# dpbriggs/Distributed-Sieve-e

Hardware: AMD Instinct MI355X
Metric: sieved integers/sec at N=1e11, 1/2/4/8 MI355X; % of LDS/HBM roofline (higher is better)
Workload: dtype u32; 1 GPU; N=1e+11 odd-only chunked sieve, P=1 spread-work chunks (one per GPU), mask resident in HBM; N=100000000000, P=1, cs=49999999999, mask_bytes_per_gpu=6250000000, parallelism=range-partition x1 (RCCL broadcast + all-reduce)

## Files before the change

distributed-sieve-e_amd/csrc/dse_wheel_geometry.h:

```cpp
#pragma once
#include <hip/hip_runtime.h>
#include <stddef.h>
#include <stdint.h>

#include <algorithm>

#include "dse_internal.h"

namespace dse {
namespace {

constexpr uint32_t KP = 1u << kWheelLogKP;
constexpr uint32_t BLOCKS = KP / 32;
constexpr uint32_t IMG_WORDS = 8 * BLOCKS;
constexpr uint32_t IMG_BYTES = 4 * IMG_WORDS;
static_assert(IMG_BYTES == KP, "a period index is its block's byte address");
#define DSE_IMG_OFF_S "32768"
constexpr uint32_t kImgOff = 32768;
#define DSE_STR2(x) #x
#define DSE_STR(x) DSE_STR2(x)
constexpr uint32_t NT = 1024;
constexpr uint32_t NW = NT / 64;
static_assert(BLOCKS % (64 * NW) == 0, "expansion blocks");
#ifndef DSE_TA
#define DSE_TA 96
#endif
constexpr uint32_t TA = DSE_TA;
#ifndef DSE_TB1
#define DSE_TB1 640
#endif
constexpr uint32_t TB1 = DSE_TB1;
#ifndef DSE_TB
#define DSE_TB 1536
#endif
constexpr uint32_t TB = DSE_TB;
static_assert(TA <= 256 && TA < TB1 && TB1 <= TB && TB <= KP / 8, "unit thresholds");
static_assert(KP / (128 * (TA + 1)) <= 10 && KP / (32 * (TB1 + 1)) <= 10, "class_marks_k covers K <= 10");
constexpr uint32_t kMidCap = TB >= 16384 ? 1920 : TB >= 8192 ? 1040 : TB >= 4096 ? 580 : 320;
constexpr uint32_t kOutWordsPerSeg = (uint32_t)(kWheelOutBits / 32);

constexpr uint32_t kQMax = 79;

constexpr uint32_t inv30_const(uint32_t q) {
  for (uint32_t x = 1; x < q; ++x)
    if ((30 * x) % q == 1) return x;
  return 0;
}
constexpr int kNG = 9;
constexpr uint32_t kGQ[kNG][3] = {{7, 11, 13}, {17, 19, 1}, {23, 29, 1}, {31, 37, 1}, {41, 43, 1},
                                  {47, 53, 1}, {59, 61, 1}, {67, 71, 1}, {73, 79, 1}};
constexpr uint32_t gmod(int g) { return kGQ[g][0] * kGQ[g][1] * kGQ[g][2]; }
constexpr uint32_t kInitWords = IMG_WORDS / NT;
constexpr uint32_t kInitRun = 32 * kInitWords;
constexpr uint32_t kExpandBlocks = BLOCKS / NW;
constexpr uint32_t kInitBlocks = kInitRun / 128 + 2;
constexpr uint32_t gdw(int g) { return ((gmod(g) + 32 * (4 * kInitBlocks + 1) + 127) / 128) * 4; }
constexpr uint32_t gbase(int g) { return g == 0 ? 0u : gbase(g - 1) + gdw(g - 1); }
constexpr uint32_t kGDW = gbase(kNG);
constexpr uint32_t kGInv30[kNG] = {inv30_const(gmod(0)), inv30_const(gmod(1)), inv30_const(gmod(2)),
                                   inv30_const(gmod(3)), inv30_const(gmod(4)), inv30_const(gmod(5)),
                                   inv30_const(gmod(6)), inv30_const(gmod(7)), inv30_const(gmod(8))};

struct InitTables {
  uint32_t w[4 * kGDW];
};
constexpr InitTables make_init_tables() {
  InitTables t{};
  for (int g = 0; g < kNG; ++g) {
    for (uint32_t j = 0; j < gdw(g) + 3; ++j) {
      uint32_t v = 0;
      for (uint32_t b = 0; b < 32; ++b) {
        const uint32_t y = 32 * j + b;
        const bool hit = y % kGQ[g][0] == 0 || y % kGQ[g][1] == 0 || (kGQ[g][2] > 1 && y % kGQ[g][2] == 0);
        v |= (uint32_t)hit << b;
      }
      for (uint32_t k = 0; k < 4; ++k)
        if (j >= k && j - k < gdw(g)) t.w[k * kGDW + gbase(g) + (j - k)] = v;
    }
  }
  return t;
}
__device__ const InitTables g_init_tables = make_init_tables();

constexpr uint32_t kLPieces = 16;
constexpr uint32_t kMaxRanges = 9;

}


struct WheelRange {
  uint64_t V0;
  uint64_t nbits;
  uint64_t KB0;
  uint64_t rho_pack;
  uint32_t* out;
  unsigned long long* count;
  uint32_t pl_pack;
  uint32_t e_iota;
  uint64_t fix;
  uint32_t seg0;
  uint16_t v0g[kNG];
  uint32_t lsh;
  uint32_t lcap[kLPieces];
  uint32_t variant;
};

struct WheelArgs {
  WheelRange r[kMaxRanges];
  uint32_t nranges;
  uint32_t nseg;
  uint32_t nthr[5];
  const uint32_t* bk_entries;
  const uint32_t* bk_start;
  const uint32_t* bk_reg0;
  const uint32_t* bk_n0;
  const unsigned long long* bk_spill;
  const uint32_t* bk_nspill;
  uint64_t bk_spill_cap;
  uint32_t bk_k0;
};
static_assert(sizeof(WheelArgs) <= 4096, "kernel arguments");
static_assert(alignof(WheelArgs) <= 8, "kernel argument layout");

namespace {

constexpr uint32_t kWaOffset = 8;

#ifndef DSE_BK_GRID
#define DSE_BK_GRID 1024
#endif
#ifndef DSE_BK_UNIT_BATCHES
#define DSE_BK_UNIT_BATCHES 4
#endif
constexpr uint32_t kBkBatchU = 16;
constexpr uint32_t kBkUnit = 64 * kBkBatchU * DSE_BK_UNIT_BATCHES;
constexpr uint32_t kBkGrid0 = DSE_BK_GRID;
#ifndef DSE_BK0_LISTS
#define DSE_BK0_LISTS 16
#endif
constexpr uint32_t kBk0Lists = DSE_BK0_LISTS;
static_assert(kBkGrid0 % kBk0Lists == 0 && 64 % kBk0Lists == 0, "band-0 bucket units");
constexpr uint32_t kKeyShift = 20;
static_assert(IMG_WORDS * 32 <= (1u << kKeyShift), "bucket entry layout");

}
}
```

distributed-sieve-e_amd/csrc/dse_wheel_kernel.h:

```cpp
#pragma once
#include <type_traits>

#include "dse_expand_bits.h"
#include "dse_wheel_geometry.h"

namespace dse {
namespace {

__device__ __forceinline__ uint32_t lds_addr(const uint32_t* p) {
  return (uint32_t)(uintptr_t)(const __attribute__((address_space(3))) uint32_t*)p;
}

__device__ __forceinline__ void lds_drain() { asm volatile("s_waitcnt lgkmcnt(0)" ::: "memory"); }

__device__ __forceinline__ uint32_t opaque(uint32_t x) {
  asm volatile("" : "+v"(x));
  return x;
}

constexpr uint32_t kBlockMask = ~31u;
#ifndef DSE_FAKE_CF_L
#define DSE_FAKE_CF_L 0
#endif
constexpr uint32_t kBlockMaskL = DSE_FAKE_CF_L ? ~127u : kBlockMask;
#ifndef DSE_FAKE_CF_INIT
#define DSE_FAKE_CF_INIT 0
#endif
#ifndef DSE_SHORT_TAIL
#define DSE_SHORT_TAIL 16
#endif
constexpr uint32_t kShortTail = DSE_SHORT_TAIL;
constexpr uint32_t odd_primes_upto(uint32_t x) {
  uint32_t c = 0;
  for (uint32_t v = 3; v <= x; v += 2) {
    bool pr = true;
    for (uint32_t d = 3; d * d <= v; d += 2)
      if (v % d == 0) { pr = false; break; }
    c += pr;
  }
  return c;
}
constexpr uint32_t kL0 = odd_primes_upto(TB);
constexpr uint32_t kLPrimeMask = 0x800FFFFFu;
static_assert(kWheelMaxPrime <= (1u << 20), "pl[] words: the L primes (odd, <= kWheelMaxPrime) are below 2^20");
__host__ __device__ constexpr uint32_t l_plan(uint32_t pmin, uint32_t pmax, uint32_t kp) {
  if (pmin > kp) return 2;
  if (pmin > kp / 2) return 1;
  const uint32_t n_min = pmax >= kp ? 0u : kp / pmax;
  const uint32_t n_all = (kp + pmin - 1) / pmin;
  return n_all - n_min <= kShortTail ? n_all << 3 : 4u | n_min << 3;
}
static_assert(l_plan(TB + 2, TB + 2, 1u << 17) < (1u << 11) && l_plan(TB + 2, TB + 2, 1u << 16) < (1u << 11),
              "the plan fits bits 20..30 of a pl[] word (bit 31: kLPrimeMask's dead-lane flag)");
static_assert(odd_primes_upto(kQMax) + kMidCap >= kL0, "the L list starts at kL0 whenever it exists");

__device__ __forceinline__ void mark_k(uint32_t pb4, uint32_t k, uint32_t one) {
  uint32_t a, b;
  asm volatile(
      "v_and_or_b32 %0, %2, %3, %4\n\t"
      "v_lshlrev_b32 %1, %2, %5\n\t"
      "ds_or_b32 %0, %1 offset:" DSE_IMG_OFF_S
      : "=&v"(a), "=&v"(b)
      : "v"(k), "s"(kBlockMask), "v"(pb4), "v"(one)
      : "memory");
}

__device__ __forceinline__ void mark_k_step(uint32_t pb4, uint32_t& k, uint32_t p, uint32_t one) {
  uint32_t a, b;
  asm volatile(
      "v_and_or_b32 %0, %2, %3, %4\n\t"
      "v_lshlrev_b32 %1, %2, %6\n\t"
      "ds_or_b32 %0, %1 offset:" DSE_IMG_OFF_S "\n\t"
      "v_add_u32 %2, %2, %5"
      : "=&v"(a), "=&v"(b), "+v"(k)
      : "s"(kBlockMask), "v"(pb4), "v"(p), "v"(one)
      : "memory");
}

__device__ __forceinline__ void mark_k_step4(uint32_t pb4, uint32_t& k, uint32_t p, uint32_t one) {
  uint32_t a0, b0, a1, b1;
  asm volatile(
      "v_and_or_b32 %0, %4, %5, %6\n\t"
      "v_lshlrev_b32 %1, %4, %8\n\t"
      "v_add_u32 %4, %4, %7\n\t"
      "ds_or_b32 %0, %1 offset:" DSE_IMG_OFF_S "\n\t"
      "v_and_or_b32 %2, %4, %5, %6\n\t"
      "v_lshlrev_b32 %3, %4, %8\n\t"
      "v_add_u32 %4, %4, %7\n\t"
      "ds_or_b32 %2, %3 offset:" DSE_IMG_OFF_S "\n\t"
      "v_and_or_b32 %0, %4, %5, %6\n\t"
      "v_lshlrev_b32 %1, %4, %8\n\t"
      "v_add_u32 %4, %4, %7\n\t"
      "ds_or_b32 %0, %1 offset:" DSE_IMG_OFF_S "\n\t"
      "v_and_or_b32 %2, %4, %5, %6\n\t"
      "v_lshlrev_b32 %3, %4, %8\n\t"
      "v_add_u32 %4, %4, %7\n\t"
      "ds_or_b32 %2, %3 offset:" DSE_IMG_OFF_S
      : "=&v"(a0), "=&v"(b0), "=&v"(a1), "=&v"(b1), "+v"(k)
      : "s"(kBlockMask), "v"(pb4), "v"(p), "v"(one)
      : "memory");
}


__device__ __forceinline__ uint32_t mark_run(uint32_t pb4, uint32_t k, uint32_t p, uint32_t n, uint32_t one) {
  uint32_t h = 0;
  for (; h + 4 <= n; h += 4) mark_k_step4(pb4, k, p, one);
  for (; h < n; ++h) mark_k_step(pb4, k, p, one);
  return k;
}

__device__ __forceinline__ void mark_tail(uint32_t pb4, uint32_t k, uint32_t p, uint32_t one) {
  uint64_t sv;
  uint32_t a, b;
  asm volatile(
      "s_mov_b64 %3, exec\n\t"
      "v_cmpx_gt_u32_e32 vcc, %5, %2\n\t"
      "s_cbranch_execz 2f\n"
      "1:\n\t"
      "v_and_or_b32 %0, %2, %6, %7\n\t"
      "v_lshlrev_b32 %1, %2, %8\n\t"
      "v_add_u32 %2, %2, %4\n\t"
      "ds_or_b32 %0, %1 offset:" DSE_IMG_OFF_S "\n\t"
      "v_cmpx_gt_u32_e32 vcc, %5, %2\n\t"
      "s_cbranch_execnz 1b\n"
      "2:\n\t"
      "s_mov_b64 exec, %3"
      : "=&v"(a), "=&v"(b), "+v"(k), "=&s"(sv)
      : "v"(p), "s"(KP), "s"(kBlockMask), "v"(pb4), "v"(one)
      : "memory", "vcc");
}

__device__ __forceinline__ void mark_at(uint32_t a, uint32_t bit) {
  asm volatile("ds_or_b32 %0, %1 offset:" DSE_IMG_OFF_S : : "v"(a), "v"(bit) : "memory");
}

template <int K>
__device__ __forceinline__ void class_marks(uint32_t pb4, uint32_t k, uint32_t p, uint32_t D, uint32_t one) {
#pragma unroll 1
  for (uint32_t r = 0; r < 32; ++r) {
    uint32_t a, b;
    asm volatile(
        "v_and_or_b32 %0, %2, %3, %4\n\t"
        "v_lshlrev_b32 %1, %2, %5\n\t"
        "ds_or_b32 %0, %1 offset:" DSE_IMG_OFF_S
        : "=&v"(a), "=&v"(b)
        : "v"(k), "s"(kBlockMask), "v"(pb4), "v"(one)
        : "memory");
#pragma unroll
    for (int t = 1; t < K; ++t) {
      a += D;
      mark_at(a, b);
    }
    k = opaque(k + p);
  }
}
__device__ __forceinline__ void class_marks_k(uint32_t K, uint32_t pb4, uint32_t k, uint32_t p, uint32_t D,
                                              uint32_t one) {
  switch (K) {
    case 0: return;
    case 1: class_marks<1>(pb4, k, p, D, one); return;
    case 2: class_marks<2>(pb4, k, p, D, one); return;
    case 3: class_marks<3>(pb4, k, p, D, one); return;
    case 4: class_marks<4>(pb4, k, p, D, one); return;
    case 5: class_marks<5>(pb4, k, p, D, one); return;
    case 6: class_marks<6>(pb4, k, p, D, one); return;
    case 7: class_marks<7>(pb4, k, p, D, one); return;
    case 8: class_marks<8>(pb4, k, p, D, one); return;
    case 9: class_marks<9>(pb4, k, p, D, one); return;
    case 10: class_marks<10>(pb4, k, p, D, one); return;
    default: __builtin_unreachable();
  }
}

__host__ __device__ __forceinline__ uint32_t mod_barrett(uint64_t x, uint32_t p, uint64_t m) {
#if defined(__HIP_DEVICE_COMPILE__)
  uint64_t q = __umul64hi(x, m);
#else
  uint64_t q = (uint64_t)(((unsigned __int128)x * m) >> 64);
#endif
  uint64_t r = x - q * p;
  if (r >= p) r -= p;
  if (r >= p) r -= p;
  return (uint32_t)r;
}

__device__ __forceinline__ uint64_t barrett_factor(uint32_t p) {
  const double dp = (double)p;
  uint64_t m = (uint64_t)(18446744073709551615.0 / dp);
  if (m > ~0ull / 2) m = ~0ull / 2;
  int64_t r = (int64_t)(~0ull - m * (uint64_t)p);
  m += (int64_t)__builtin_floor((double)r / dp);
  r = (int64_t)(~0ull - m * (uint64_t)p);
  while (r < 0) { --m; r += p; }
  while (r >= (int64_t)p) { ++m; r -= p; }
  return m;
}

__device__ __forceinline__ float fast_rcp(float x) { return __builtin_amdgcn_rcpf(x); }

__device__ __forceinline__ uint32_t div_ceil_small(uint32_t t, uint32_t p, float invp) {
  uint32_t q = (uint32_t)((float)t * invp);
  q = q * p > t ? q - 1 : q;
  q = (q + 1) * p <= t ? q + 1 : q;
  return q + (q * p != t ? 1u : 0u);
}

__device__ __forceinline__ uint32_t div_small(uint32_t t, uint32_t p, float invp) {
  uint32_t q = (uint32_t)((float)t * invp);
  q = q * p > t ? q - 1 : q;
  q = (q + 1) * p <= t ? q + 1 : q;
  return q;
}

__device__ __forceinline__ uint32_t mulmod_small(uint32_t x, uint32_t y, uint32_t p, float invp) {
  const uint32_t xy = x * y;
  uint32_t q = (uint32_t)((float)xy * invp);
  int32_t r = (int32_t)(xy - q * p);
  r = r < 0 ? r + (int32_t)p : r;
  r = r < 0 ? r + (int32_t)p : r;
  r = r >= (int32_t)p ? r - (int32_t)p : r;
  r = r >= (int32_t)p ? r - (int32_t)p : r;
  return (uint32_t)r;
}

__host__ __device__ __forceinline__ uint64_t inv30_of(uint64_t p) {
  constexpr uint64_t T = (14ull << 0) | (8ull << 12) | (9ull << 20) | (11ull << 24) | (3ull << 32) | (5ull << 36) |
                         (6ull << 44) | (0ull << 56);
  const uint32_t r = (uint32_t)(p % 30u);
  const uint64_t a = 2 * ((T >> (4 * (r >> 1))) & 15) + 1;
  return (p * a + 1) / 30;
}

__device__ __forceinline__ uint32_t plane_first(uint32_t Xs, uint32_t rho, uint32_t p, uint32_t inv30,
                                                float invp) {
  uint32_t t = Xs + rho;
  t = t >= p ? t - p : t;
  const uint32_t u = t ? p - t : 0u;
  return mulmod_small(u, inv30, p, invp);
}

__device__ __forceinline__ uint32_t first_at_or_after(uint32_t kp, uint32_t start, uint32_t p, float invp) {
  if (start <= kp) return kp;
  return kp + p * div_ceil_small(start - kp, p, invp);
}

__device__ __forceinline__ uint32_t kmin_for(uint32_t D, uint32_t rho) {
  return D > rho ? (D - rho + 29u) / 30u : 0u;
}


template <int K>
__device__ __forceinline__ void a_classes(uint32_t pb4, uint32_t k, uint32_t p, uint32_t one) {
  const uint32_t D = p << 8;
#pragma unroll 1
  for (uint32_t r = 0; r < 32; ++r) {
    uint32_t a, bit;
    asm volatile(
        "v_and_or_b32 %0, %2, %3, %4\n\t"
        "v_lshlrev_b32 %1, %2, %5"
        : "=&v"(a), "=&v"(bit)
        : "v"(k), "s"(kBlockMask), "v"(pb4), "v"(one));
#pragma unroll
    for (int t = 0; t < K; ++t) {
      mark_at(a, bit);
      a += D;
    }
    mark_at(a, bit);
    k = opaque(k + p);
  }
}

struct MidRes {
  uint32_t* x;
  const uint32_t* inc;
  bool have;
};
__device__ __forceinline__ uint32_t mid_residue(const MidRes& mr, uint32_t i, uint32_t p, uint64_t m, uint64_t Vs,
                                                bool writer) {
  const uint32_t xs = mr.have ? mr.x[i] : mod_barrett(Vs, p, m);
  if (writer) {
    const uint32_t t = xs + mr.inc[i];
    mr.x[i] = min(t, t - p);
  }
  return xs;
}

__device__ __forceinline__ void unit_A(uint32_t img0, uint32_t pi, uint64_t m, const MidRes& mr, uint32_t idx,
                                       uint64_t Vs, uint64_t rho_pack, uint32_t lane, uint32_t one) {
  const uint32_t p = pi & 0xFFFFu, inv30 = pi >> 16;
  const uint64_t p2 = (uint64_t)p * p;
  const uint32_t Xs = __builtin_amdgcn_readfirstlane(mid_residue(mr, idx, p, m, Vs, lane == 0));
  const float invp = fast_rcp((float)p);
  const uint32_t pl = lane & 7, c = lane >> 3;
  const uint32_t rho = (uint32_t)(rho_pack >> (5 * pl)) & 31u;
  const uint32_t kp = plane_first(Xs, rho, p, inv30, invp);
  const uint32_t pb4 = img0 + 4 * pl;
  const uint32_t k = kp + 32 * c * p;
  if (p2 <= Vs) {
    switch (KP / (256 * p)) {
      case 1: a_classes<1>(pb4, k, p, one); return;
      case 2: a_classes<2>(pb4, k, p, one); return;
      case 3: a_classes<3>(pb4, k, p, one); return;
      case 4: a_classes<4>(pb4, k, p, one); return;
      case 5: a_classes<5>(pb4, k, p, one); return;
      case 6: a_classes<6>(pb4, k, p, one); return;
      case 7: a_classes<7>(pb4, k, p, one); return;
      default: __builtin_unreachable();
    }
  }
  const uint32_t kmin = kmin_for((uint32_t)(p2 - Vs), rho);
  for (uint32_t r = 0; r < 32; ++r)
    for (uint32_t kk = k + r * p; kk < KP; kk += 256 * p)
      if (kk >= kmin) mark_k(pb4, kk, one);
}

__device__ __forceinline__ void unit_B1(uint32_t img0, const uint32_t* __restrict__ s_mid_p,
                                        const uint64_t* __restrict__ s_mid_m, const MidRes& mr, uint32_t j0,
                                        uint32_t nj, uint64_t Vs, uint64_t rho_pack, uint32_t lane, uint32_t one) {
  const uint32_t h = lane >> 5, pl = lane & 7, j = (lane >> 3) & 3;
  if (h >= nj) return;
  const uint32_t pi = s_mid_p[j0 + h];
  const uint32_t p = pi & 0xFFFFu, inv30 = pi >> 16;
  const uint64_t m = s_mid_m[j0 + h];
  const float invp = fast_rcp((float)p);
  const uint32_t rho = (uint32_t)(rho_pack >> (5 * pl)) & 31u;
  const uint32_t kp = plane_first(mid_residue(mr, j0 + h, p, m, Vs, (lane & 31) == 0), rho, p, inv30, invp);
  const uint32_t pb4 = img0 + 4 * pl;
  uint32_t k = kp + 32 * j * p;
  const uint64_t p2 = (uint64_t)p * p;
  if (p2 > Vs) {
    const uint32_t kmin = kmin_for((uint32_t)min(p2 - Vs, (uint64_t)0xFFFFFFFFu), rho);
    for (; k < KP; k += 96 * p)
      for (uint32_t r = 0; r < 32 && k < KP; ++r, k += p)
        if (k >= kmin) mark_k(pb4, k, one);
    return;
  }
  const uint32_t pmax = __builtin_amdgcn_readlane(p, nj == 2 ? 32 : 0);
  const uint32_t tf = (KP / pmax) / 128;
  class_marks_k(tf, pb4, k, p, 128 * p, one);
  k += tf * (128 * p);
  const uint32_t pmin = __builtin_amdgcn_readfirstlane(p);
  const uint32_t n_all = __builtin_amdgcn_readfirstlane(div_ceil_small(KP, pmin, fast_rcp((float)pmin)));
  for (uint32_t base = 128 * tf; base < n_all; base += 128) {
    mark_run(pb4, k, p, min(32u, n_all - base), one);
    k += 128 * p;
  }
}

__device__ __forceinline__ void unit_B2(uint32_t img0, const uint32_t* __restrict__ s_mid_p,
                                        const uint64_t* __restrict__ s_mid_m, const MidRes& mr, uint32_t j0,
                                        uint32_t nj, uint64_t Vs, uint64_t Vend, uint64_t rho_pack, uint32_t lane,
                                        uint32_t one) {
  const uint32_t pl = lane & 7, jp = lane >> 3;
  const bool valid = jp < nj;
  const uint32_t pi = s_mid_p[valid ? j0 + jp : j0];
  const uint32_t p = pi & 0xFFFFu, inv30 = pi >> 16;
  const uint64_t m = s_mid_m[valid ? j0 + jp : j0];
  const float invp = fast_rcp((float)p);
  const uint32_t rho = (uint32_t)(rho_pack >> (5 * pl)) & 31u;
  uint32_t k = plane_first(mid_residue(mr, valid ? j0 + jp : j0, p, m, Vs, valid && pl == 0), rho, p, inv30, invp);
  const uint64_t p2 = (uint64_t)p * p;
  const bool slow = p2 > Vs;
  if (slow) k = p2 >= Vend ? KP : first_at_or_after(k, kmin_for((uint32_t)(p2 - Vs), rho), p, invp);
  const uint32_t pmax = __builtin_amdgcn_readfirstlane(s_mid_p[j0 + nj - 1]) & 0xFFFFu;
  const bool any_slow = __builtin_amdgcn_ballot_w64(slow) != 0;
  const uint32_t n_u = any_slow ? 0u : KP / pmax;
  const uint32_t pb4 = img0 + 4 * pl;
  if (!valid) return;
  const uint32_t K = n_u / 32;
  class_marks_k(K, pb4, k, p, 32 * p, one);
  k += K * (32 * p);
  if (any_slow) {
    mark_tail(pb4, mark_run(pb4, k, p, n_u - 32 * K, one), p, one);
    return;
  }
  const uint32_t pmin = __builtin_amdgcn_readfirstlane(s_mid_p[j0]) & 0xFFFFu;
  const uint32_t n_all = __builtin_amdgcn_readfirstlane(div_ceil_small(KP, pmin, fast_rcp((float)pmin)));
  mark_run(pb4, k, p, n_all - 32 * K, one);
}

struct LargeOps {
  uint32_t p;
  uint64_t m;
  uint32_t a[8];
};

__device__ __forceinline__ void load_L(LargeOps& o, const uint32_t* __restrict__ P, const uint64_t* __restrict__ M,
                                       const uint32_t* __restrict__ A, uint32_t il, uint32_t np, bool need_m) {
  const uint32_t ic = min(il, np - 1);
  o.p = il < np ? *reinterpret_cast<const uint32_t*>(reinterpret_cast<const char*>(P) + (ic << 2)) : 0xFFFFFFFFu;
  o.m = need_m ? M[ic] : 0ull;
  const uint4* row = reinterpret_cast<const uint4*>(reinterpret_cast<const char*>(A) + (ic << 5));
  const uint4 lo = row[0], hi = row[1];
  o.a[0] = lo.x; o.a[1] = lo.y; o.a[2] = lo.z; o.a[3] = lo.w;
  o.a[4] = hi.x; o.a[5] = hi.y; o.a[6] = hi.z; o.a[7] = hi.w;
}

__device__ __forceinline__ void undef_ops(LargeOps& o) {
  asm volatile("" : "=v"(o.p), "=v"(o.m), "=v"(o.a[0]), "=v"(o.a[1]), "=v"(o.a[2]), "=v"(o.a[3]), "=v"(o.a[4]),
               "=v"(o.a[5]), "=v"(o.a[6]), "=v"(o.a[7]));
}

__device__ __forceinline__ void mark_entry(uint32_t img0, uint32_t e, uint32_t one) {
  uint32_t a, b;
  asm volatile(
      "v_lshrrev_b32 %0, 3, %2\n\t"
      "v_and_or_b32 %0, %0, -4, %4\n\t"
      "v_lshlrev_b32 %1, %2, %3\n\t"
      "ds_or_b32 %0, %1 offset:" DSE_IMG_OFF_S
      : "=&v"(a), "=&v"(b)
      : "v"(e), "v"(one), "v"(img0)
      : "memory");
}

constexpr uint64_t kQuotBits = 22;
constexpr uint64_t kQuotErr38 = (1ull << (38 - 22)) / (TB + 1) + 1;
static_assert((1ull << 32) / (TB + 1) < (1ull << kQuotBits), "Kb < 2^32: float quotient within 1 (and < 2^24 for __umul24)");
static_assert((kQuotErr38 + 2) * kWheelMaxPrime < (1ull << 31), "Kb < 2^38: the rest Kb - q p must be exact in int32");
static_assert(kWheelMaxPrime < (1ull << 23), "__mul24 / __umul24 operands and float-exact p");
static_assert((uint64_t)(kWheelMaxPrime + 1) * (kWheelMaxPrime + 1) / 30 < (1ull << 38),
              "ranges without bucketed primes never need the Barrett path (unit_L<false>)");

__device__ __forceinline__ uint32_t kb_mod_p_f32(uint32_t kb, uint32_t p, float invp) {
  const uint32_t q = (uint32_t)((float)kb * invp);
  uint32_t qp;
  asm("v_mul_u32_u24 %0, %1, %2" : "=v"(qp) : "v"(q), "v"(p));
  uint32_t x = kb - qp;
  x = min(x, x + p);
  return min(x, x - p);
}

__device__ __forceinline__ uint32_t kb_mod_p_f38(uint64_t Kb, uint32_t p, float invp) {
  const uint32_t q = (uint32_t)((float)Kb * invp);
  const int32_t r = (int32_t)((uint32_t)Kb - q * p);
  const int32_t q2 = (int32_t)((float)r * invp);
  uint32_t x = (uint32_t)(r - __mul24(q2, (int32_t)p));
  x = min(x, x + p);
  return min(x, x - p);
}

template <bool BARRETT>
__device__ __forceinline__ uint32_t kb_mod_p(uint64_t Kb, uint32_t p, float invp, uint64_t m) {
  if (Kb < (1ull << 32)) return kb_mod_p_f32((uint32_t)Kb, p, invp);
  if (!BARRETT || Kb < (1ull << 38)) return kb_mod_p_f38(Kb, p, invp);
  return mod_barrett(Kb, p, m);
}

struct PlaneSteps {
  uint32_t pb[8];
  uint32_t ne[8];
  uint32_t one;
};

__device__ __forceinline__ uint32_t plane_start(uint32_t a, uint32_t nKbm, uint32_t ne, uint32_t p) {
  uint32_t t, u;
  asm("v_add3_u32 %0, %2, %3, %4\n\t"
      "v_add_u32 %1, %0, %5\n\t"
      "v_min_u32 %0, %0, %1"
      : "=&v"(t), "=&v"(u)
      : "v"(a), "v"(nKbm), "v"(ne), "v"(p));
  return t;
}

#define DSE_PLANE_START(A, NE)                                       \
  "v_add3_u32 %0, " A ", %15, " NE "\n\t"  \
  "v_add_u32 %1, %0, %16\n\t"                                        \
  "v_min_u32 %0, %0, %1\n\t"
#define DSE_PLANE_MARK(PB)               \
  "v_and_or_b32 %1, %0, %17, " PB "\n\t" \
  "v_lshlrev_b32 %2, %0, %18\n\t"        \
  "ds_or_b32 %1, %2 offset:" DSE_IMG_OFF_S "\n\t"
#define DSE_PLANE_NEXT "v_add_u32 %0, %0, %16\n\t"
template <int NM>
__device__ __forceinline__ void start_marks4(const uint32_t* a, const uint32_t* ne, const uint32_t* pb, uint32_t nKbm,
                                             uint32_t p, uint32_t one) {
  uint32_t t, u, b;
  if (NM == 1)
    asm volatile(
        DSE_PLANE_START("%3", "%7") DSE_PLANE_MARK("%11")
        DSE_PLANE_START("%4", "%8") DSE_PLANE_MARK("%12")
        DSE_PLANE_START("%5", "%9") DSE_PLANE_MARK("%13")
        DSE_PLANE_START("%6", "%10") DSE_PLANE_MARK("%14")
        : "=&v"(t), "=&v"(u), "=&v"(b)
        : "v"(a[0]), "v"(a[1]), "v"(a[2]), "v"(a[3]), "v"(ne[0]), "v"(ne[1]), "v"(ne[2]), "v"(ne[3]), "v"(pb[0]),
          "v"(pb[1]), "v"(pb[2]), "v"(pb[3]), "v"(nKbm), "v"(p), "s"(kBlockMaskL), "v"(one)
        : "memory");
  else
    asm volatile(
        DSE_PLANE_START("%3", "%7") DSE_PLANE_MARK("%11") DSE_PLANE_NEXT DSE_PLANE_MARK("%11")
        DSE_PLANE_START("%4", "%8") DSE_PLANE_MARK("%12") DSE_PLANE_NEXT DSE_PLANE_MARK("%12")
        DSE_PLANE_START("%5", "%9") DSE_PLANE_MARK("%13") DSE_PLANE_NEXT DSE_PLANE_MARK("%13")
        DSE_PLANE_START("%6", "%10") DSE_PLANE_MARK("%14") DSE_PLANE_NEXT DSE_PLANE_MARK("%14")
        : "=&v"(t), "=&v"(u), "=&v"(b)
        : "v"(a[0]), "v"(a[1]), "v"(a[2]), "v"(a[3]), "v"(ne[0]), "v"(ne[1]), "v"(ne[2]), "v"(ne[3]), "v"(pb[0]),
          "v"(pb[1]), "v"(pb[2]), "v"(pb[3]), "v"(nKbm), "v"(p), "s"(kBlockMaskL), "v"(one)
        : "memory");
}

#ifndef DSE_LOCKSTEP
#define DSE_LOCKSTEP 1
#endif
#define DSE_MARK8_ONE(A, B, K, PB)                   \
  "v_and_or_b32 " A ", " K ", %21, " PB "\n\t"     \
  "v_lshlrev_b32 " B ", " K ", %22\n\t"             \
  "v_add_u32 " K ", " K ", %20\n\t"                 \
  "ds_or_b32 " A ", " B " offset:" DSE_IMG_OFF_S "\n\t"
__device__ __forceinline__ void mark8(uint32_t (&k)[8], const uint32_t* pb, uint32_t p, uint32_t one) {
  uint32_t a0, b0, a1, b1;
  asm volatile(DSE_MARK8_ONE("%0", "%1", "%4", "%12") DSE_MARK8_ONE("%2", "%3", "%5", "%13")
                   DSE_MARK8_ONE("%0", "%1", "%6", "%14") DSE_MARK8_ONE("%2", "%3", "%7", "%15")
                       DSE_MARK8_ONE("%0", "%1", "%8", "%16") DSE_MARK8_ONE("%2", "%3", "%9", "%17")
                           DSE_MARK8_ONE("%0", "%1", "%10", "%18") DSE_MARK8_ONE("%2", "%3", "%11", "%19")
               : "=&v"(a0), "=&v"(b0), "=&v"(a1), "=&v"(b1), "+v"(k[0]), "+v"(k[1]), "+v"(k[2]), "+v"(k[3]),
                 "+v"(k[4]), "+v"(k[5]), "+v"(k[6]), "+v"(k[7])
               : "v"(pb[0]), "v"(pb[1]), "v"(pb[2]), "v"(pb[3]), "v"(pb[4]), "v"(pb[5]), "v"(pb[6]), "v"(pb[7]),
                 "v"(p), "s"(kBlockMaskL), "v"(one)
               : "memory");
}

template <int MODE, bool TAIL = false>
__device__ __forceinline__ void unit_L_fast(const LargeOps& o, uint32_t p, uint32_t nKbm, const PlaneSteps& ps,
                                            uint32_t n_run) {
  if (MODE != 0) {
    constexpr int NM = MODE == 2 ? 1 : 2;
    start_marks4<NM>(o.a, ps.ne, ps.pb, nKbm, p, ps.one);
    start_marks4<NM>(o.a + 4, ps.ne + 4, ps.pb + 4, nKbm, p, ps.one);
    return;
  }
#if DSE_LOCKSTEP
  if (!TAIL) {
    uint32_t kk[8];
#pragma unroll
    for (uint32_t q = 0; q < 8; ++q) kk[q] = plane_start(o.a[q], nKbm, ps.ne[q], p);
#pragma unroll 1
    for (uint32_t h = 0; h < n_run; ++h) mark8(kk, ps.pb, p, ps.one);
    return;
  }
#endif
#pragma unroll
  for (uint32_t q = 0; q < 8; ++q) {
    const uint32_t kk = plane_start(o.a[q], nKbm, ps.ne[q], p);
    const uint32_t pb4 = ps.pb[q];
    const uint32_t k = mark_run(pb4, kk, p, n_run, ps.one);
    if (TAIL) mark_tail(pb4, k, p, ps.one);
  }
}

template <bool BARRETT>
__device__ __forceinline__ void unit_L(const LargeOps& o, uint64_t Vs, uint64_t Vend, uint64_t Kb,
                                       const PlaneSteps& ps, uint32_t pl_rot, const uint64_t* rho_pack_p,
                                       uint32_t sqrt_vs) {
  const uint32_t p = o.p & kLPrimeMask;
  const float invp = fast_rcp((float)p);
  const uint32_t kbm = kb_mod_p<BARRETT>(Kb, p, invp, o.m);
  const uint32_t nKbm = 0u - kbm;
  const uint32_t pmax = __builtin_amdgcn_readlane(p, 63);
  const bool none = pmax > sqrt_vs;
  if (!none) {
    const uint32_t plan = (uint32_t)__builtin_amdgcn_readfirstlane(o.p) >> 20;
    const uint32_t n_run = plan >> 3;
    if ((plan & 3) == 2) unit_L_fast<2>(o, p, nKbm, ps, 0);
    else if ((plan & 3) == 1) unit_L_fast<1>(o, p, nKbm, ps, 0);
    else if (!(plan & 4)) unit_L_fast<0>(o, p, nKbm, ps, n_run);
    else unit_L_fast<0, true>(o, p, nKbm, ps, n_run);
    return;
  }
  const uint32_t pmin = __builtin_amdgcn_readfirstlane(p);
  const uint64_t p2 = (uint64_t)p * p;
  const bool live = p2 < Vend;
  const bool slow = p2 > Vs;
  const uint32_t D = slow && live ? (uint32_t)(p2 - Vs) : 0u;
  if (!live) return;
  const uint64_t rho_pack = *(volatile const uint64_t*)rho_pack_p;
#pragma unroll
  for (uint32_t q = 0; q < 8; ++q) {
    uint32_t kk = plane_start(o.a[q], nKbm, ps.ne[q], p);
    if (slow) {
      const uint32_t pl = (pl_rot >> (3 * q)) & 7u;
      const uint32_t rho = (uint32_t)(rho_pack >> (5 * pl)) & 31u;
      const uint32_t kmin = kmin_for(D, rho);
      if (kmin > kk) {
        const uint32_t d = kmin - kk;
        uint32_t qd = (uint32_t)((float)d * invp);
        while (qd * p < d) ++qd;
        while (qd > 0 && (qd - 1) * p >= d) --qd;
        kk += qd * p;
      }
    }
    const uint32_t pb4 = ps.pb[q];
    if (pmin > KP / 2) {
      mark_k(pb4, kk, ps.one);
      mark_k(pb4, kk + p, ps.one);
    } else {
      for (; kk < KP; kk += p) mark_k(pb4, kk, ps.one);
    }
  }
}

struct WheelLdsLow {
  uint64_t mid_m[kMidCap];
  uint32_t mid_p[kMidCap];
  uint32_t mid_x[kMidCap];
  uint32_t mid_inc[kMidCap];
  uint32_t x_seg;
  uint4 itab[kGDW];
  uint32_t thr[5];
  uint32_t ctr;
  unsigned long long rcnt[kMaxRanges];
};
static_assert(sizeof(WheelLdsLow) <= kImgOff, "LDS below the image");
struct WheelLds : WheelLdsLow {
  uint8_t pad[kImgOff - sizeof(WheelLdsLow)];
  uint32_t img[IMG_WORDS];
};
static_assert(sizeof(WheelLds) == kImgOff + IMG_BYTES, "the image ends the allocation");

template <bool BK>
__global__ __launch_bounds__(NT) void wheel_segments_kernel(const void* __restrict__ table, WheelArgs wa) {
  __shared__ WheelLds lds;
  uint64_t* const s_mid_m = lds.mid_m;
  uint32_t* const s_mid_p = lds.mid_p;
  uint32_t* const s_thr = lds.thr;

  const TableHeader* th = reinterpret_cast<const TableHeader*>(table);
  const uint32_t np = th->count;
  const uint32_t* __restrict__ P = reinterpret_cast<const uint32_t*>(reinterpret_cast<const char*>(table) + 16);
  const uint64_t* __restrict__ M =
      reinterpret_cast<const uint64_t*>(reinterpret_cast<const char*>(table) + table_m_offset(th->cap));
  const uint32_t* __restrict__ A =
      reinterpret_cast<const uint32_t*>(reinterpret_cast<const char*>(table) + table_a_offset(th->cap));
  const uint32_t* __restrict__ PL = reinterpret_cast<const uint32_t*>(reinterpret_cast<const char*>(table) +
                                                                    table_l_offset(th->cap)) +
                                    (kWheelLogKP == 17 ? 0u : th->cap);

#if defined(DSE_PAD_NOPS) && DSE_PAD_NOPS > 0
  asm volatile(".rept " DSE_STR(DSE_PAD_NOPS) "\n\ts_nop 0\n\t.endr");
#endif
  const uint32_t tid = threadIdx.x, lane_id = tid & 63, wave = tid >> 6;

  if (tid == 0) {
    s_thr[0] = min(wa.nthr[0], np);
    s_thr[1] = min(wa.nthr[1], np);
    s_thr[2] = min(wa.nthr[2], np);
    s_thr[3] = min(min(wa.nthr[3], np), s_thr[0] + kMidCap);
    s_thr[2] = min(s_thr[2], s_thr[3]);
    s_thr[4] = max(s_thr[3], min(wa.nthr[4], np));
    lds.ctr = 0;
    lds.x_seg = ~0u;
  }
  if (tid < kMaxRanges) lds.rcnt[tid] = 0;
  for (uint32_t idx = tid; idx < 4 * kGDW; idx += NT) reinterpret_cast<uint32_t*>(lds.itab)[idx] = g_init_tables.w[idx];
  __syncthreads();
  const uint32_t i_mid0 = s_thr[0], i_midB = s_thr[1], i_midB2 = s_thr[2], i_mid1 = s_thr[3];
  for (uint32_t i = tid; i < i_mid1 - i_mid0; i += NT) {
    const uint32_t q = P[i_mid0 + i];
    s_mid_p[i] = q | ((uint32_t)inv30_of(q) << 16);
    s_mid_m[i] = M[i_mid0 + i];
    lds.mid_inc[i] = (uint32_t)(((uint64_t)gridDim.x * kWheelSpan) % q);
  }
  const uint32_t nA = i_midB - i_mid0;
  const uint32_t n_mid = i_mid1 - i_mid0;
  const uint32_t n_b1 = i_midB2 - i_mid0;
  const uint32_t nB1 = (i_midB2 - i_midB + 1) / 2;
  const uint32_t nB2 = (i_mid1 - i_midB2 + 7) / 8;
  const uint32_t i_big = s_thr[4];
  constexpr uint32_t kLU = 128;
  const uint32_t n1 = nA + nB1 + nB2;

  const uint32_t nseg = wa.nseg;
  const uint32_t grid = gridDim.x;
  const uint32_t T = blockIdx.x < nseg ? (nseg - 1 - blockIdx.x) / grid + 1 : 0u;
  auto range_of = [&](uint32_t g) -> uint32_t {
    uint32_t r = 0;
    for (uint32_t i = 1; i < wa.nranges; ++i) r = g >= wa.r[i].seg0 ? i : r;
    return r;
  };

  auto init_segment = [&](uint32_t* __restrict__ img, uint32_t g_seg) {
    const WheelRange& rg = wa.r[range_of(g_seg)];
    const uint64_t s = g_seg - rg.seg0;
    uint32_t lane = lane_id;
    asm volatile("" : "+v"(lane));
    const uint32_t pl = lane & 7, q = 8 * wave + (lane >> 3);
    const uint32_t rho = (uint32_t)(rg.rho_pack >> (5 * pl)) & 31u;
    constexpr uint32_t R = kInitWords;
    static_assert(R % 4 == 0, "staggered init runs");
    const uint32_t j = q & 3;
    const uint32_t b0 = 4 * R * (q >> 2) + (R + 1) * j;
    const uint32_t k0 = 32 * b0;
    constexpr uint32_t H = 16;
    static_assert(R % H == 0 && H % 4 == 0, "init passes");
    uint32_t boff[kNG], bsh[kNG];
    const uint32_t rho_o = opaque(rho), k0_o = opaque(k0);
#pragma unroll
    for (int g = 0; g < kNG; ++g) {
      const uint32_t Mg = gmod(g);
      const uint32_t wg = (uint32_t)(kWheelSpan % Mg);
      const uint32_t sg = (uint32_t)(s % Mg);
      const uint32_t x = ((uint32_t)rg.v0g[g] + sg * wg + rho_o) % Mg;
      const uint32_t o = (k0_o + x * kGInv30[g]) % Mg;
      const uint32_t d0 = o >> 5, kc = d0 & 3;
      boff[g] = (kc * kGDW + gbase(g) + d0 - kc) / 4;
#if DSE_FAKE_CF_INIT
      boff[g] = gbase(g) / 4 + (lane & 15u);
#endif
      bsh[g] = o & 31;
    }
    uint32_t* const wp = img + 8 * b0 + pl;
#pragma unroll
    for (uint32_t h = 0; h < R; h += H) {
      uint32_t acc[H];
#pragma unroll
      for (uint32_t r = 0; r < H; ++r) acc[r] = 0;
#pragma unroll
      for (int g = 0; g < kNG; ++g) {
        const uint4* bp = lds.itab + boff[g] + h / 4;
        uint32_t blk[H + 4];
#pragma unroll
        for (uint32_t b = 0; b < H / 4 + 1; ++b) {
          const uint4 v = bp[b];
          blk[4 * b] = v.x; blk[4 * b + 1] = v.y; blk[4 * b + 2] = v.z; blk[4 * b + 3] = v.w;
        }
#pragma unroll
        for (uint32_t r = 0; r < H; ++r) acc[r] |= __builtin_amdgcn_alignbit(blk[r + 1], blk[r], bsh[g]);
        asm volatile("" ::: "memory");
      }
#pragma unroll
      for (uint32_t r = 0; r < H; ++r) {
        if (h + r >= R - 3 && j == 3) continue;
        wp[8 * (h + r)] = acc[r];
      }
    }
    if (j != 3) {
      uint32_t acc = 0;
#pragma unroll
      for (int g = 0; g < kNG; ++g) {
        const uint4* bp = lds.itab + boff[g] + R / 4;
        const uint4 v = bp[0];
        acc |= __builtin_amdgcn_alignbit(v.y, v.x, bsh[g]);
      }
      wp[8 * R] = acc;
    }
  };

  auto expand_blocks = [&](const uint32_t* __restrict__ img, uint32_t g_seg, uint32_t ri, auto vt) {
    constexpr int VT = decltype(vt)::value;
    const WheelRange& rg = wa.r[ri];
    const uint64_t s = g_seg - rg.seg0;
    const uint64_t out_words = 2ull * ((rg.nbits + 63) / 64);
    uint32_t* __restrict__ out = rg.out;
    uint32_t my_count = 0;
    uint32_t lane = lane_id;
    asm volatile("" : "+v"(lane));
    const uint32_t l = lane & 31;
    const uint32_t gsub = (l >= 4 && l < 12) || (l >= 16 && l < 20) || l >= 28;
    const uint32_t m = l < 4 ? l : l < 12 ? l - 4 : l < 20 ? l - 8 : l < 28 ? l - 12 : l - 16;
    const uint32_t bl = 16 * (2 * (lane >> 5) + gsub) + m;
    const uint64_t seg_word0 = s * (uint64_t)kOutWordsPerSeg;
    const ExpandMasks masks = expand_masks();
#pragma unroll 1
    for (uint32_t t = 0; t < kExpandBlocks / 64; ++t) {
      const uint32_t blk = kExpandBlocks * wave + 64 * t + bl;
      const uint4* rp = reinterpret_cast<const uint4*>(img + 8 * blk);
      const uint4 lo = rp[0], hi = rp[1];
      uint32_t W[8] = {lo.x, lo.y, lo.z, lo.w, hi.x, hi.y, hi.z, hi.w};
      uint32_t n_comp = 0;
#pragma unroll
      for (int j = 0; j < 8; ++j) n_comp += __popc(W[j]);
      uint32_t o[15];
      expand_block<VT>(W, o, masks);
      const uint64_t w0 = seg_word0 + 15ull * blk;
      if (s == 0 && blk == 0) {
        o[0] |= (uint32_t)rg.fix;
        o[1] |= (uint32_t)(rg.fix >> 32);
      }
      const uint64_t bit0 = 32ull * w0;
      if (bit0 + 480 <= rg.nbits) {
        uint32_t cnt = 0;
        if (s == 0 && blk == 0) {
#pragma unroll
          for (int w = 0; w < 15; ++w) cnt += __popc(o[w]);
        } else {
          cnt = 256u - n_comp;
        }
        my_count += cnt;
        if (out) {
#pragma unroll
          for (int w = 0; w < 15; ++w) out[w0 + w] = o[w];
        }
      } else {
        const uint32_t rem = bit0 >= rg.nbits ? 0u : (uint32_t)(rg.nbits - bit0);
        uint32_t cnt = 0;
#pragma unroll
        for (int w = 0; w < 15; ++w) {
          const uint32_t b = 32u * w;
          o[w] = b >= rem ? 0u : (rem - b >= 32 ? o[w] : o[w] & ((1u << (rem - b)) - 1u));
          cnt += __popc(o[w]);
        }
        my_count += cnt;
        if (out) {
#pragma unroll
          for (int w = 0; w < 15; ++w)
            if (w0 + w < out_words) out[w0 + w] = o[w];
        }
      }
    }
#pragma unroll
    for (int o = 32; o > 0; o >>= 1) my_count += __shfl_xor(my_count, o);
    if (lane == 0 && my_count) atomicAdd(&lds.rcnt[ri], (unsigned long long)my_count);
  };
  auto expand_segment = [&](const uint32_t* __restrict__ img, uint32_t g_seg) {
    const uint32_t ri = range_of(g_seg);
    switch (__builtin_amdgcn_readfirstlane(wa.r[ri].variant)) {
#define DSE_EXPAND_CASE(V) \
  case V: expand_blocks(img, g_seg, ri, std::integral_constant<int, V>{}); break;
      DSE_EXPAND_CASE(0) DSE_EXPAND_CASE(1) DSE_EXPAND_CASE(2) DSE_EXPAND_CASE(3) DSE_EXPAND_CASE(4)
      DSE_EXPAND_CASE(5) DSE_EXPAND_CASE(6) DSE_EXPAND_CASE(7) DSE_EXPAND_CASE(8) DSE_EXPAND_CASE(9)
      DSE_EXPAND_CASE(10) DSE_EXPAND_CASE(11) DSE_EXPAND_CASE(12) DSE_EXPAND_CASE(13) DSE_EXPAND_CASE(14)
#undef DSE_EXPAND_CASE
      default: break;
    }
  };

  auto mark_segment = [&](uint32_t* __restrict__ img, uint32_t g_seg) {
    const WheelRange& rg = wa.r[range_of(g_seg)];
    const uint64_t s = g_seg - rg.seg0;
    const uint64_t Vs = rg.V0 + s * kWheelSpan;
    const uint64_t Vend = Vs + kWheelSpan;
    uint32_t lane = lane_id;
    asm volatile("" : "+v"(lane));
    const uint32_t img0 = lds_addr(img) - kImgOff;
    const uint32_t one = opaque(1u);
    uint32_t bk_b0 = 0, bk_b1 = 0, n0u = 0, n1u = 0, n3 = 0;
    if (BK) {
      n0u = wa.bk_k0 ? kBkGrid0 / kBk0Lists : 0u;
      bk_b0 = wa.bk_start[s];
      bk_b1 = wa.bk_start[s + 1];
      n1u = (bk_b1 - bk_b0 + kBkUnit - 1) / kBkUnit;
      n3 = n0u + n1u + (wa.bk_k0 && *wa.bk_nspill ? 1u : 0u);
    }
    const uint64_t* rho_pack_p = reinterpret_cast<const uint64_t*>(
        (const char*)__builtin_amdgcn_kernarg_segment_ptr() + kWaOffset +
        range_of(g_seg) * sizeof(WheelRange) + offsetof(WheelRange, rho_pack));
    uint32_t sqrt_vs = (uint32_t)__builtin_sqrt((double)Vs);
    while ((uint64_t)sqrt_vs * sqrt_vs > Vs) --sqrt_vs;
    while ((uint64_t)(sqrt_vs + 1) * (sqrt_vs + 1) <= Vs) ++sqrt_vs;
    sqrt_vs = __builtin_amdgcn_readfirstlane(sqrt_vs);
    uint32_t sqrt_ve = (uint32_t)__builtin_sqrt((double)(Vend - 1));
    while ((uint64_t)sqrt_ve * sqrt_ve > Vend - 1) --sqrt_ve;
    while ((uint64_t)(sqrt_ve + 1) * (sqrt_ve + 1) <= Vend - 1) ++sqrt_ve;
    sqrt_ve = __builtin_amdgcn_readfirstlane(sqrt_ve);
    const uint32_t rot = (i_mid1 + lane) & 7;
    const uint32_t pl_rot = ((rg.pl_pack >> (3 * rot)) | (rg.pl_pack << (24 - 3 * rot))) & 0xFFFFFFu;
    const uint32_t e_rot = ((rg.e_iota >> rot) | (rg.e_iota << (8 - rot))) & 0xFFu;
    PlaneSteps ps;
    ps.one = one;
#pragma unroll
    for (uint32_t q = 0; q < 8; ++q) {
      ps.pb[q] = img0 + 4 * ((pl_rot >> (3 * q)) & 7u) + (DSE_FAKE_CF_L ? ((lane_id >> 3) & 3u) << 5 : 0u);
      ps.ne[q] = 0u - ((e_rot >> q) & 1u);
    }
    const uint64_t Kb = rg.KB0 + s * (uint64_t)KP;
    const bool need_m = BK && Kb >= (1ull << 38);
    MidRes mr;
    mr.x = lds.mid_x;
    mr.inc = lds.mid_inc;
    mr.have = __builtin_amdgcn_readfirstlane(lds.x_seg) == g_seg;
    const uint32_t i_live = max(i_mid1, min(i_big, rg.lcap[min((uint32_t)(s >> rg.lsh), kLPieces - 1)]));
    const uint32_t n2 = (i_live - i_mid1 + kLU - 1) / kLU;
    const uint32_t n_int = min(n1, n2), n_all = n1 + n2;
    const uint32_t ctr_addr = lds_addr(&lds.ctr);
    auto claim = [&]() -> uint32_t {
      uint32_t j = 0;
      if (lane == 0) asm volatile("ds_add_rtn_u32 %0, %1, %2" : "=v"(j) : "v"(ctr_addr), "v"(1u) : "memory");
      return j;
    };
    auto claimed = [&](uint32_t j) -> uint32_t {
      asm volatile("s_waitcnt lgkmcnt(0)" : "+v"(j)::"memory");
      return __builtin_amdgcn_readlane(j, 0);
    };
    auto is_l = [&](uint32_t u) -> bool { return u < 2 * n_int ? (u & 1) != 0 : n2 > n1; };
    auto idx_of = [&](uint32_t u) -> uint32_t { return u < 2 * n_int ? u >> 1 : u - n_int; };
    const uint32_t mb = min(n3, n_all), n_q = n_all + n3;
    auto unit_of = [&](uint32_t q) -> uint32_t {
      if (q < 2 * mb) return (q & 1) ? ~0u : q >> 1;
      return n3 > n_all ? ~0u : q - mb;
    };
    auto bk_of = [&](uint32_t q) -> uint32_t { return q < 2 * mb ? q >> 1 : q - mb; };
    constexpr uint32_t kIdx = (1u << 30) - 1;
    auto decode = [&](uint32_t q) -> uint32_t {
      if (q >= n_q) return ~0u;
      const uint32_t u = unit_of(q);
      if (u == ~0u) return 2u << 30 | bk_of(q);
      return (is_l(u) ? 1u << 30 : 0u) | idx_of(u);
    };
    LargeOps cur, nxt;
    LargeOps cur1, nxt1;
    uint32_t d_nxt = decode(claimed(claim()));
    if ((d_nxt >> 30) == 1) {
      load_L(nxt, PL, M, A, i_mid1 + kLU * (d_nxt & kIdx) + lane, i_big, need_m);
      load_L(nxt1, PL, M, A, i_mid1 + kLU * (d_nxt & kIdx) + 64 + lane, i_big, need_m);
    }
    uint32_t d_after = decode(claimed(claim()));
    asm volatile("" ::"v"(nxt.p), "v"(nxt.a[0]), "v"(nxt.a[1]), "v"(nxt.a[2]), "v"(nxt.a[3]), "v"(nxt.a[4]),
                 "v"(nxt.a[5]), "v"(nxt.a[6]), "v"(nxt.a[7]), "v"(nxt1.p), "v"(nxt1.a[0]), "v"(nxt1.a[1]),
                 "v"(nxt1.a[2]), "v"(nxt1.a[3]), "v"(nxt1.a[4]), "v"(nxt1.a[5]), "v"(nxt1.a[6]), "v"(nxt1.a[7]));
    for (;;) {
      cur = nxt;
      cur1 = nxt1;
      undef_ops(nxt);
      undef_ops(nxt1);
      const uint32_t d_cur = d_nxt;
      d_nxt = d_after;
      if (d_cur == ~0u) break;
      const uint32_t c2 = claim();
      if ((d_nxt >> 30) == 1) {
        load_L(nxt, PL, M, A, i_mid1 + kLU * (d_nxt & kIdx) + lane, i_big, need_m);
        load_L(nxt1, PL, M, A, i_mid1 + kLU * (d_nxt & kIdx) + 64 + lane, i_big, need_m);
      }
      if (BK && (d_cur >> 30) == 2) {
        const uint32_t bu = d_cur & kIdx;
        if (bu < n0u) {
          const uint64_t li0 = s * (uint64_t)kBkGrid0 + bu * kBk0Lists;
          const uint32_t nl = lane < kBk0Lists ? wa.bk_n0[li0 + lane] : 0u;
#pragma unroll 1
          for (uint32_t g = 0; g < kBk0Lists; g += 4) {
            uint32_t n[4], nmax = 0;
            const uint32_t* __restrict__ r[4];
#pragma unroll
            for (uint32_t l = 0; l < 4; ++l) {
              n[l] = min((uint32_t)__builtin_amdgcn_readlane((int)nl, (int)(g + l)), wa.bk_k0);
              r[l] = wa.bk_reg0 + ((uint64_t)(bu * kBk0Lists + g + l) * wa.nseg + s) * wa.bk_k0;
              nmax = max(nmax, n[l]);
            }
            for (uint32_t o = lane; o < nmax + lane; o += 256) {
              uint32_t e[16];
#pragma unroll
              for (uint32_t l = 0; l < 4; ++l)
#pragma unroll
                for (uint32_t t = 0; t < 4; ++t)
                  e[4 * l + t] = o + 64 * t < n[l] ? __builtin_nontemporal_load(r[l] + o + 64 * t) : 0u;
#pragma unroll
              for (uint32_t l = 0; l < 4; ++l)
#pragma unroll
                for (uint32_t t = 0; t < 4; ++t)
                  if (o + 64 * t < n[l]) mark_entry(img0, e[4 * l + t], one);
            }
          }
        } else if (bu < n0u + n1u) {
          const uint32_t beg = bk_b0 + (bu - n0u) * kBkUnit, end = min(bk_b1, beg + kBkUnit);
          for (uint32_t j = beg + lane; j < end; j += 64 * kBkBatchU) {
            uint32_t e[kBkBatchU];
#pragma unroll
            for (uint32_t t = 0; t < kBkBatchU; ++t)
              e[t] = j + 64 * t < end ? __builtin_nontemporal_load(wa.bk_entries + j + 64 * t) : 0u;
#pragma unroll
            for (uint32_t t = 0; t < kBkBatchU; ++t)
              if (j + 64 * t < end) mark_entry(img0, e[t], one);
          }
        } else {
          const uint32_t ns = (uint32_t)min((uint64_t)*wa.bk_nspill, wa.bk_spill_cap);
          for (uint32_t j = lane; j < ns; j += 64) {
            const unsigned long long v = wa.bk_spill[j];
            if ((uint32_t)(v >> 32) == (uint32_t)s) mark_entry(img0, (uint32_t)v, one);
          }
        }
        d_after = decode(claimed(c2));
        continue;
      }
      const uint32_t k = d_cur & kIdx;
      if ((d_cur >> 30) == 0) {
        if (k < nA) {
          const uint32_t pi = __builtin_amdgcn_readfirstlane(s_mid_p[k]);
          const uint32_t p = pi & 0xFFFFu;
          const uint64_t m = ((uint64_t)(uint32_t)__builtin_amdgcn_readfirstlane((uint32_t)(s_mid_m[k] >> 32)) << 32) |
                             (uint32_t)__builtin_amdgcn_readfirstlane((uint32_t)s_mid_m[k]);
          if ((uint64_t)p * p < Vend) unit_A(img0, pi, m, mr, k, Vs, rg.rho_pack, lane, one);
        } else if (k < nA + nB1) {
          const uint32_t j0 = nA + (k - nA) * 2;
          const uint32_t pf = __builtin_amdgcn_readfirstlane(s_mid_p[j0]) & 0xFFFFu;
          if ((uint64_t)pf * pf < Vend)
            unit_B1(img0, s_mid_p, s_mid_m, mr, j0, min(2u, n_b1 - j0), Vs, rg.rho_pack, lane, one);
        } else {
          const uint32_t j0 = n_b1 + (k - nA - nB1) * 8;
          const uint32_t pf = __builtin_amdgcn_readfirstlane(s_mid_p[j0]) & 0xFFFFu;
          if ((uint64_t)pf * pf < Vend)
            unit_B2(img0, s_mid_p, s_mid_m, mr, j0, min(8u, n_mid - j0), Vs, Vend, rg.rho_pack, lane, one);
        }
      } else {
        const uint32_t p0 = __builtin_amdgcn_readfirstlane(cur.p) & kLPrimeMask;
        if (p0 <= sqrt_ve) unit_L<BK>(cur, Vs, Vend, Kb, ps, pl_rot, rho_pack_p, sqrt_vs);
        const uint32_t p1 = __builtin_amdgcn_readfirstlane(cur1.p) & kLPrimeMask;
        if (p1 <= sqrt_ve) unit_L<BK>(cur1, Vs, Vend, Kb, ps, pl_rot, rho_pack_p, sqrt_vs);
      }
      d_after = decode(claimed(c2));
    }
  };

  if (T > 0) init_segment(lds.img, blockIdx.x);
  __syncthreads();
  for (uint32_t t = 0; t < T; ++t) {
    const uint32_t s = blockIdx.x + t * grid;
    mark_segment(lds.img, s);
    lds_drain();
    __syncthreads();
    expand_segment(lds.img, s);
    if (t + 1 < T) init_segment(lds.img, s + grid);
    if (tid == 0) {
      lds.ctr = 0;
      const uint32_t r0 = range_of(s), r1 = range_of(s + grid);
      const uint64_t Vs = wa.r[r0].V0 + (uint64_t)(s - wa.r[r0].seg0) * kWheelSpan;
      lds.x_seg = t + 1 < T && r1 == r0 && Vs >= (uint64_t)TB * TB ? s + grid : ~0u;
    }
    __syncthreads();
  }

  if (tid < wa.nranges && lds.rcnt[tid]) atomicAdd(wa.r[tid].count, lds.rcnt[tid]);
}

template <bool BK>
hipError_t launch_wheel(const void* table, const WheelArgs& wa, int num_cus, hipStream_t stream) {
  if (wa.nseg == 0) return hipSuccess;
  const uint32_t grid = wheel_grid(wa.nseg, num_cus);
  hipLaunchKernelGGL(wheel_segments_kernel<BK>, dim3(grid), dim3(NT), 0, stream, table, wa);
  return hipGetLastError();
}

}
}
```

Before: 18300 billion integers/s.

## Unroll class marking and regroup B2 units to four primes, two lanes each

```diff
diff --git a/distributed-sieve-e_amd/csrc/dse_wheel_geometry.h b/distributed-sieve-e_amd/csrc/dse_wheel_geometry.h
--- a/distributed-sieve-e_amd/csrc/dse_wheel_geometry.h
+++ b/distributed-sieve-e_amd/csrc/dse_wheel_geometry.h
@@ -35,7 +35,9 @@
 #endif
 constexpr uint32_t TB = DSE_TB;
 static_assert(TA <= 256 && TA < TB1 && TB1 <= TB && TB <= KP / 8, "unit thresholds");
-static_assert(KP / (128 * (TA + 1)) <= 10 && KP / (32 * (TB1 + 1)) <= 10, "class_marks_k covers K <= 10");
+constexpr uint32_t kClassMarksMax = 11;
+static_assert((KP - 1) / (128 * (TA + 1)) + 1 <= kClassMarksMax && (KP - 1) / (64 * (TB1 + 1)) + 1 <= kClassMarksMax,
+              "class_marks_k covers K <= kClassMarksMax");
 constexpr uint32_t kMidCap = TB >= 16384 ? 1920 : TB >= 8192 ? 1040 : TB >= 4096 ? 580 : 320;
 constexpr uint32_t kOutWordsPerSeg = (uint32_t)(kWheelOutBits / 32);
 
diff --git a/distributed-sieve-e_amd/csrc/dse_wheel_kernel.h b/distributed-sieve-e_amd/csrc/dse_wheel_kernel.h
--- a/distributed-sieve-e_amd/csrc/dse_wheel_kernel.h
+++ b/distributed-sieve-e_amd/csrc/dse_wheel_kernel.h
@@ -134,24 +134,24 @@
   asm volatile("ds_or_b32 %0, %1 offset:" DSE_IMG_OFF_S : : "v"(a), "v"(bit) : "memory");
 }
 
+#define DSE_CLASS(A, B)                                  \
+  "v_and_or_b32 " A ", %4, %5, %6\n\t"                   \
+  "v_lshlrev_b32 " B ", %4, %7\n\t"                      \
+  "v_add_u32 %4, %4, %8\n\t"                             \
+  "ds_or_b32 " A ", " B " offset:" DSE_IMG_OFF_S "\n\t"  \
+  ".rept %c10\n\t"                                       \
+  "v_add_u32 " A ", " A ", %9\n\t"                       \
+  "ds_or_b32 " A ", " B " offset:" DSE_IMG_OFF_S "\n\t"  \
+  ".endr\n\t"
 template <int K>
 __device__ __forceinline__ void class_marks(uint32_t pb4, uint32_t k, uint32_t p, uint32_t D, uint32_t one) {
 #pragma unroll 1
-  for (uint32_t r = 0; r < 32; ++r) {
-    uint32_t a, b;
-    asm volatile(
-        "v_and_or_b32 %0, %2, %3, %4\n\t"
-        "v_lshlrev_b32 %1, %2, %5\n\t"
-        "ds_or_b32 %0, %1 offset:" DSE_IMG_OFF_S
-        : "=&v"(a), "=&v"(b)
-        : "v"(k), "s"(kBlockMask), "v"(pb4), "v"(one)
-        : "memory");
-#pragma unroll
-    for (int t = 1; t < K; ++t) {
-      a += D;
-      mark_at(a, b);
-    }
-    k = opaque(k + p);
+  for (uint32_t r = 0; r < 32; r += 4) {
+    uint32_t a0, b0, a1, b1;
+    asm volatile(".rept 2\n\t" DSE_CLASS("%0", "%1") DSE_CLASS("%2", "%3") ".endr"
+                 : "=&v"(a0), "=&v"(b0), "=&v"(a1), "=&v"(b1), "+v"(k)
+                 : "s"(kBlockMask), "v"(pb4), "v"(one), "v"(p), "v"(D), "n"(K - 1)
+                 : "memory");
   }
 }
 __device__ __forceinline__ void class_marks_k(uint32_t K, uint32_t pb4, uint32_t k, uint32_t p, uint32_t D,
@@ -168,6 +168,7 @@
     case 8: class_marks<8>(pb4, k, p, D, one); return;
     case 9: class_marks<9>(pb4, k, p, D, one); return;
     case 10: class_marks<10>(pb4, k, p, D, one); return;
+    case 11: class_marks<11>(pb4, k, p, D, one); return;
     default: __builtin_unreachable();
   }
 }
@@ -335,48 +336,36 @@
         if (k >= kmin) mark_k(pb4, k, one);
     return;
   }
-  const uint32_t pmax = __builtin_amdgcn_readlane(p, nj == 2 ? 32 : 0);
-  const uint32_t tf = (KP / pmax) / 128;
-  class_marks_k(tf, pb4, k, p, 128 * p, one);
-  k += tf * (128 * p);
   const uint32_t pmin = __builtin_amdgcn_readfirstlane(p);
-  const uint32_t n_all = __builtin_amdgcn_readfirstlane(div_ceil_small(KP, pmin, fast_rcp((float)pmin)));
-  for (uint32_t base = 128 * tf; base < n_all; base += 128) {
-    mark_run(pb4, k, p, min(32u, n_all - base), one);
-    k += 128 * p;
-  }
+  const uint32_t T = __builtin_amdgcn_readfirstlane(div_small(KP - 1, pmin, fast_rcp((float)pmin))) / 128 + 1;
+  class_marks_k(T, pb4, k, p, 128 * p, one);
 }
 
 __device__ __forceinline__ void unit_B2(uint32_t img0, const uint32_t* __restrict__ s_mid_p,
                                         const uint64_t* __restrict__ s_mid_m, const MidRes& mr, uint32_t j0,
-                                        uint32_t nj, uint64_t Vs, uint64_t Vend, uint64_t rho_pack, uint32_t lane,
-                                        uint32_t one) {
-  const uint32_t pl = lane & 7, jp = lane >> 3;
-  const bool valid = jp < nj;
-  const uint32_t pi = s_mid_p[valid ? j0 + jp : j0];
+                                        uint32_t nj, uint64_t Vs, uint64_t rho_pack, uint32_t lane, uint32_t one) {
+  const uint32_t h = lane >> 4, pl = lane & 7, j = (lane >> 3) & 1;
+  if (h >= nj) return;
+  const uint32_t pi = s_mid_p[j0 + h];
   const uint32_t p = pi & 0xFFFFu, inv30 = pi >> 16;
-  const uint64_t m = s_mid_m[valid ? j0 + jp : j0];
+  const uint64_t m = s_mid_m[j0 + h];
   const float invp = fast_rcp((float)p);
   const uint32_t rho = (uint32_t)(rho_pack >> (5 * pl)) & 31u;
-  uint32_t k = plane_first(mid_residue(mr, valid ? j0 + jp : j0, p, m, Vs, valid && pl == 0), rho, p, inv30, invp);
-  const uint64_t p2 = (uint64_t)p * p;
-  const bool slow = p2 > Vs;
-  if (slow) k = p2 >= Vend ? KP : first_at_or_after(k, kmin_for((uint32_t)(p2 - Vs), rho), p, invp);
+  const uint32_t kp = plane_first(mid_residue(mr, j0 + h, p, m, Vs, (lane & 15) == 0), rho, p, inv30, invp);
+  const uint32_t pb4 = img0 + 4 * pl;
+  uint32_t k = kp + 32 * j * p;
   const uint32_t pmax = __builtin_amdgcn_readfirstlane(s_mid_p[j0 + nj - 1]) & 0xFFFFu;
-  const bool any_slow = __builtin_amdgcn_ballot_w64(slow) != 0;
-  const uint32_t n_u = any_slow ? 0u : KP / pmax;
-  const uint32_t pb4 = img0 + 4 * pl;
-  if (!valid) return;
-  const uint32_t K = n_u / 32;
-  class_marks_k(K, pb4, k, p, 32 * p, one);
-  k += K * (32 * p);
-  if (any_slow) {
-    mark_tail(pb4, mark_run(pb4, k, p, n_u - 32 * K, one), p, one);
+  if ((uint64_t)pmax * pmax > Vs) {
+    const uint64_t p2 = (uint64_t)p * p;
+    const uint32_t kmin = p2 > Vs ? kmin_for((uint32_t)min(p2 - Vs, (uint64_t)0xFFFFFFFFu), rho) : 0u;
+    for (; k < KP; k += 32 * p)
+      for (uint32_t r = 0; r < 32 && k < KP; ++r, k += p)
+        if (k >= kmin) mark_k(pb4, k, one);
     return;
   }
-  const uint32_t pmin = __builtin_amdgcn_readfirstlane(s_mid_p[j0]) & 0xFFFFu;
-  const uint32_t n_all = __builtin_amdgcn_readfirstlane(div_ceil_small(KP, pmin, fast_rcp((float)pmin)));
-  mark_run(pb4, k, p, n_all - 32 * K, one);
+  const uint32_t pmin = __builtin_amdgcn_readfirstlane(p);
+  const uint32_t T2 = __builtin_amdgcn_readfirstlane(div_small(KP - 1, pmin, fast_rcp((float)pmin))) / 64 + 1;
+  class_marks_k(T2, pb4, k, p, 64 * p, one);
 }
 
 struct LargeOps {
@@ -662,7 +651,7 @@
   const uint32_t n_mid = i_mid1 - i_mid0;
   const uint32_t n_b1 = i_midB2 - i_mid0;
   const uint32_t nB1 = (i_midB2 - i_midB + 1) / 2;
-  const uint32_t nB2 = (i_mid1 - i_midB2 + 7) / 8;
+  const uint32_t nB2 = (i_mid1 - i_midB2 + 3) / 4;
   const uint32_t i_big = s_thr[4];
   constexpr uint32_t kLU = 128;
   const uint32_t n1 = nA + nB1 + nB2;
@@ -982,10 +971,10 @@
           if ((uint64_t)pf * pf < Vend)
             unit_B1(img0, s_mid_p, s_mid_m, mr, j0, min(2u, n_b1 - j0), Vs, rg.rho_pack, lane, one);
         } else {
-          const uint32_t j0 = n_b1 + (k - nA - nB1) * 8;
+          const uint32_t j0 = n_b1 + (k - nA - nB1) * 4;
           const uint32_t pf = __builtin_amdgcn_readfirstlane(s_mid_p[j0]) & 0xFFFFu;
           if ((uint64_t)pf * pf < Vend)
-            unit_B2(img0, s_mid_p, s_mid_m, mr, j0, min(8u, n_mid - j0), Vs, Vend, rg.rho_pack, lane, one);
+            unit_B2(img0, s_mid_p, s_mid_m, mr, j0, min(4u, n_mid - j0), Vs, rg.rho_pack, lane, one);
         }
       } else {
         const uint32_t p0 = __builtin_amdgcn_readfirstlane(cur.p) & kLPrimeMask;
```

Result: faster. 18670 billion integers/s, median of 6 (+2.0%).
